# rssalessio/TZDDPC

Hardware: AMD Instinct MI355X
Metric: MPC steps/sec (batched trajectories), double-integrator N=20 (higher is better)
Workload: dtype f64

## Files before the change

### include/tzddpc.h

```cpp
#ifndef TZDDPC_H
#define TZDDPC_H

#include <stdint.h>

#ifdef __cplusplus
extern "C" {
#endif

#define TZ_ABI_VERSION 4

typedef enum tz_status {
  TZ_OK = 0,
  TZ_ERR_INVALID = -1,
  TZ_ERR_HIP = -2,
  TZ_ERR_UNSUPPORTED = -3
} tz_status;

enum {
  TZ_SOLVED = 0,
  TZ_MAX_ITER = 1,
  TZ_NUMERICAL = 2,
  TZ_INFEASIBLE = 3,
};

// ... 35 lines not shown
  int32_t pmax;
  const double* absCKpow;
  const double* absKCKpow;
  const int32_t* power;
  int32_t max_iter;
  double tol;
  double reg;
  double step_frac;
  const int32_t* shift_var;
  const int32_t* shift_row;
  const double* shift_xscale;
  const double* shift_lscale;
  const double* rec_c0;
  const double* rec_x0;
  const double* rec_y;
  int32_t plan_flags;
} tz_problem_desc;

enum {
  TZ_PLAN_UNFUSED = 1,
  TZ_PLAN_GENERAL_CHOLESKY = 2,
  TZ_PLAN_ITEM_GRAM = 4,
  TZ_PLAN_NO_STAIRCASE = 8,
  TZ_PLAN_ELL_PRODUCTS = 16
};

typedef struct tz_problem tz_problem;

int tz_abi_version(void);
const char* tz_last_error(void);
int tz_device_count(int* count);

int tz_identify_batch(int device, int32_t B, int32_t T, int32_t n, int32_t m, const double* u, const double* x,
                      const double* w_center, const double* K, int32_t k_shared,
                      double* C, double* s, double* sK, double* CK, int32_t* status, int mem);

int tz_specrad_batch(int device, int32_t S, int32_t n, int32_t ngen, const double* M0, const double* H, const double* beta,
                     double* rho, int32_t* status);
int tz_adversary_batch(int device, int32_t S, int32_t n, int32_t ngen, const double* M0, const double* H, const double* beta0,
                       int32_t max_iter, double* beta, double* fro, int32_t* steps);

typedef struct tz_genstack_desc {
  int32_t n, m, N, nseg;
  const int32_t* seg_ptr;
  const int32_t* src;
  const double* m0;
  const double* M;
// ... 33 lines not shown
               const double* A_true, const double* B_true, double* u_out, double* cost, int32_t* status);

int tz_problem_store_start(tz_problem* p, const double* xbar0, const double* e0);

int tz_problem_set_warm_shift(tz_problem* p, int32_t policy);
int tz_problem_set_warm_quiet(tz_problem* p, int32_t quiet_steps);

int tz_problem_set_stopping(tz_problem* p, double res_factor, double mu_factor);

int tz_problem_set_warm_push(tz_problem* p, double floor, double gain, double cap);

int tz_problem_reset_warm(tz_problem* p);

int tz_timing_enable(tz_problem* p, int enable);
int tz_timing_get(tz_problem* p, int kernel, double* total_ms, int64_t* launches);
int tz_ipm_work_get(tz_problem* p, int64_t* factorizations, int64_t* trajectory_solves, int64_t* max_factorizations_one_trajectory);

int tz_ipm_plan_info(tz_problem* p, int64_t* mfma_gram_per_iter, int64_t* mfma_chol_per_iter,
                     int64_t* mfma_issued_per_iter, int64_t* lds_bytes, int64_t* patch_bytes);

int tz_problem_plan_get(tz_problem* p, int32_t* fused, int32_t* one_wave_cholesky, int32_t* superstep_gram, int32_t* staircase,
                        int32_t* toeplitz);

int tz_debug_fetch(tz_problem* p, int32_t b, int what, double* out, int32_t capacity);

#ifdef __cplusplus
}
#endif
#endif
```

### tzddpc_amd/csrc/tz_ipm.hip.h

```cpp
#pragma once

#define TZ_MINWAVES 4
#define TZ_RLEV_CARRY_MAX 2
#ifndef TZ_RLEV_GATE
#define TZ_RLEV_GATE 1e6
#endif
#define TZ_SEED_VIOL_MAX 0.1
#define TZ_QROW 17
#define TZ_QSTR (4 * TZ_QROW)
struct IpmItem { int I0, q0, nq, kptr, klen; };

struct TzEll { int L, VL; const TzEllEnt* ent; const int* seg; const double* val; const unsigned short* idx; };
typedef __attribute__((address_space(1))) const char* tz_gptr;
typedef __attribute__((address_space(1))) const tz_d2* tz_gd2ptr;
__device__ inline double tz_ell_walk(const char* base_, unsigned lo, int L, unsigned stride, const double* in) {
  double a0 = 0.0, a1 = 0.0;
  const char* b = reinterpret_cast<const char*>(in);
  tz_gptr base = (tz_gptr)base_;
  int e = 0;
  for (; e + 3 < L; e += 4) {
    tz_gptr q0 = base, q1 = base + stride, q2 = base + 2 * (size_t)stride, q3 = base + 3 * (size_t)stride;
    asm volatile("" : "+s"(q0), "+s"(q1), "+s"(q2), "+s"(q3));
    const tz_d2 r0 = *(tz_gd2ptr)(q0 + lo), r1 = *(tz_gd2ptr)(q1 + lo), r2 = *(tz_gd2ptr)(q2 + lo), r3 = *(tz_gd2ptr)(q3 + lo);
    base += 4 * (size_t)stride;
// ... 35 lines not shown
  const int* smask;
  const double* q; const double* h;
  const int* prestatus;
  double* x; double* s; double* lam;
  int* status; int* iters;
  const int* prev_status;
  int* status_copy;
  int max_iter; double tol, reg, step_frac;
  double inv_mi;
  double mu_floor, tol_loose, step_frac_retry;
  double mu_tol;
  double tol_res;
  int warm_steps;
  int nell;
  int ntube;
  int shift_policy;
  int* shift_state;
  int shift_quiet;
  const int* sx; const int* sr; const double* sxs; const double* sls;
  int TS, ntile, gu;
  const struct TzGUnit* gunits; const int* gunit_ptr;
  int chol1;
  int ksplit;
  int warm; double warm_floor;
  double warm_gain, warm_cap;
  double aff_thr, aff_mu;
  unsigned long long* work;
  unsigned long long* prof;
  FuseParams F;
};

enum { PH_FORM = 0, PH_CHOL = 1, PH_SOLVE = 2, PH_GEMVT = 3, PH_GEMV = 4, PH_ELEM = 5, PH_TOTAL = 6, PH_CH_UPD = 8, PH_CH_DIAG = 9, PH_CH_PANEL = 10, PH_CH_BAR = 11, PH_PROLOGUE = 12, PH_EPILOGUE = 13, PH_GRAM_LOOP = 14, PH_GRAM_RED = 15, PH_GRAM_BAR = 16, PH_GRAM_RMW = 17, PH_TUBE = 18, PH_WARM = 19, PH_TOP = 20, PH_STEP = 21,
       PH_RD_A = 22, PH_RD_B = 23, PH_RD_C = 24, PH_EPI_A = 25, PH_EPI_B = 26, PH_MAPS_Q = 27, PH_WARM_A = 28, PH_WARM_B = 29, PH_TEST = 30, PH_T1 = 31, PH_T2 = 32, PH_T3 = 33, PH_COUNT = 34 };

__device__ inline int tz_qprefix(int I) {
  int a = I >> 2, b = I & 3;
  return (a + 1) * (2 * a + b);
}
__device__ inline int tz_hidx(int r, int c) {
  int I = r >> 2, J = c >> 2;
  return (tz_qprefix(I) + (J >> 2)) * TZ_QSTR + TZ_QROW * (r & 3) + 4 * (J & 3) + (c & 3);
}

__device__ inline int tz_tid() {
  int v = threadIdx.x;
  asm volatile("" : "+v"(v));
// ... 249 lines not shown
#pragma unroll
    for (int ii = 0; ii < 4; ++ii) {
      const int I = I0 + ii;
      if (I >= Tz) continue;
#pragma unroll
      for (int nn = 0; nn < 2; ++nn) {
        const int q = q0 + nn;
        if (nn >= nq || q > (I >> 2)) continue;
        const int r = 4 * I + i, c = 4 * (4 * q + blk) + j;
        double v = acc[ii][nn];
        if (c < p.nzp) v += p.P[(size_t)r * p.nzp + c];
        if (r == c) v = (r < p.nz) ? v + p.reg : 1.0;
        Hq[(tz_qprefix(I) + q) * TZ_QSTR + TZ_QROW * i + 4 * blk + j] = v;
      }
    }
  }
}

#define TZ_KS_TZ 10
__device__ inline double tz_sel4(int blk, double v0, double v1, double v2, double v3) {
  const double a = (blk & 1) ? v1 : v0, b = (blk & 1) ? v3 : v2;
  return (blk & 2) ? b : a;
}
struct TzGStage { double v[TZ_KS_TZ]; double w; int m; };

template <int N>
__device__ inline double tz_row_ror(double v) {
  const unsigned long long u = __builtin_bit_cast(unsigned long long, v);
  constexpr int ctrl = 0x120 + N;
  const unsigned lo = (unsigned)__builtin_amdgcn_mov_dpp((int)(unsigned)u, ctrl, 0xf, 0xf, true);
  const unsigned hi = (unsigned)__builtin_amdgcn_mov_dpp((int)(unsigned)(u >> 32), ctrl, 0xf, 0xf, true);
  return __builtin_bit_cast(double, ((unsigned long long)hi << 32) | lo);
}

template <int R0, int R1>
__device__ inline void tz_gram_rows(const IpmParams& p, double* Hq, const double* Pq, const double* wv, const int* sm, const int h, unsigned long long* pacc) {
  unsigned long long tq0 = pacc ? __builtin_amdgcn_s_memtime() : 0;
  const int lane = tz_tid() & 63;
  const int k = lane >> 4, blk = (lane >> 2) & 3, ij = lane & 3;
  const int Tz = p.Tz, Kc = p.Kc, S = (Kc + 3) >> 2;
  const unsigned rowbytes = (unsigned)(Tz + 1) * 128u;
  const char* gp = (const char*)p.Gp + (unsigned)(4 * k + ij) * 8u;
  double acc[R1 - R0][R1];
#pragma unroll
  for (int a = 0; a < R1 - R0; ++a)
#pragma unroll
    for (int J = 0; J < R1; ++J) acc[a][J] = 0.0;
  auto load = [&](int s, TzGStage& st) {
    int kc = 4 * s + blk; kc = (kc < Kc) ? kc : Kc;
    st.m = sm[s < S ? s : S];
    st.w = wv[4 * kc + k];
    const char* prow = gp + (size_t)kc * rowbytes;
#pragma unroll
    for (int J = 0; J < R1; ++J) st.v[J] = tz_ld_pinned((const double*)(prow + (unsigned)(J < Tz ? J : Tz) * 128u));
  };
  auto mma = [&](const TzGStage& st) {
    const int m = __builtin_amdgcn_readfirstlane(st.m);
#pragma unroll
    for (int I = R0; I < R1; ++I) {
      if ((m >> I) & 1) {
        const double a = st.v[I] * st.w;
#pragma unroll
        for (int J = 0; J <= I; ++J)
          if ((m >> J) & 1) acc[I - R0][J] = __builtin_amdgcn_mfma_f64_4x4x4f64(a, st.v[J], acc[I - R0][J], 0, 0, 0);
      }
    }
  };
  TzGStage s0, s1;
  load(h, s0);
  for (int s = h; s < S; s += 4) {
    load(s + 2, s1); mma(s0);
    load(s + 4, s0); mma(s1);
  }
  if (pacc) { unsigned long long t1 = __builtin_amdgcn_s_memtime(); pacc[PH_GRAM_LOOP] += t1 - tq0; tq0 = t1; }
  const int i = lane >> 4, j = lane & 3;
#pragma unroll
  for (int a = 0; a < R1 - R0; ++a)
#pragma unroll
    for (int J = 0; J < R1; ++J)
      if (J <= a + R0) { double v = acc[a][J]; v += tz_row_ror<4>(v); v += tz_row_ror<8>(v); acc[a][J] = v; }
  for (int hh = 0; hh < 2; ++hh) {
    if (h == hh) {
#pragma unroll
      for (int I = R0; I < R1; ++I) {
        if (I >= Tz) continue;
#pragma unroll
        for (int q = 0; q <= (I >> 2); ++q) {
          const double v0 = acc[I - R0][4 * q];
          const double v1 = (4 * q + 1 <= I) ? acc[I - R0][(4 * q + 1 <= I) ? 4 * q + 1 : 0] : 0.0;
          const double v2 = (4 * q + 2 <= I) ? acc[I - R0][(4 * q + 2 <= I) ? 4 * q + 2 : 0] : 0.0;
          const double v3 = (4 * q + 3 <= I) ? acc[I - R0][(4 * q + 3 <= I) ? 4 * q + 3 : 0] : 0.0;
          const int idx = (tz_qprefix(I) + q) * TZ_QSTR + TZ_QROW * i + 4 * blk + j;
          Hq[idx] = tz_sel4(blk, v0, v1, v2, v3) + ((hh == 0) ? Pq[idx] : Hq[idx]);
        }
      }
    }
    if (pacc) { unsigned long long t1 = __builtin_amdgcn_s_memtime(); pacc[hh == 0 ? PH_GRAM_RED : PH_GRAM_RMW] += t1 - tq0; tq0 = t1; }
    if (hh == 0) __syncthreads();
    if (pacc && hh == 0) { unsigned long long t1 = __builtin_amdgcn_s_memtime(); pacc[PH_GRAM_BAR] += t1 - tq0; tq0 = t1; }
  }
}

__device__ inline void tz_form_H_ksplit(const IpmParams& p, double* Hq, const double* Pq, const double* wv, const int* sm, unsigned long long* pacc) {
  const int wave = __builtin_amdgcn_readfirstlane(threadIdx.x >> 6);
  const int g = wave >> 1, h = wave & 1;
  if (p.Tz > 7) { if (g == 0) tz_gram_rows<0, 7>(p, Hq, Pq, wv, sm, h, pacc); else tz_gram_rows<7, 10>(p, Hq, Pq, wv, sm, h, pacc); }
  else          { if (g == 0) tz_gram_rows<0, 5>(p, Hq, Pq, wv, sm, h, pacc); else tz_gram_rows<5, 7>(p, Hq, Pq, wv, sm, h, pacc); }
}

__device__ inline void tz_gram(const IpmParams& p, double* Hq, const double* Pq, const double* wv, const int* kl, unsigned long long* pacc = nullptr) {
  if (p.ksplit) tz_form_H_ksplit(p, Hq, Pq, wv, kl, pacc);
  else tz_form_H(p, Hq, wv, kl);
}

__device__ inline void tz_sqrt_rsqrt(double d, double& sq, double& rs) {
  double y = __builtin_amdgcn_rsq(d);
  double g = d * y, h = 0.5 * y;
  double r = __builtin_fma(-h, g, 0.5);
  g = __builtin_fma(g, r, g); h = __builtin_fma(h, r, h);
  const double e = __builtin_fma(-g, g, d);
  g = __builtin_fma(e, h, g);
  double inv = h + h;
  const double e2 = __builtin_fma(-g, inv, 1.0);
  inv = __builtin_fma(e2, inv, inv);
  sq = g; rs = inv;
}

__device__ inline double tz_recip(double x) {
  double y = __builtin_amdgcn_rcp(x);
  y = __builtin_fma(__builtin_fma(-x, y, 1.0), y, y);
// ... 377 lines not shown
  double* thl = red + 34 + (p.nklist + 1) / 2;
  double* stl = thl + p.F.ntheta;
  double* pl = stl + 4 * TZ_NMAX;
  double* tbl = pl + p.nell;
  double* Pq = tbl + p.ntube;
  constexpr bool PARK = (MINW == 4);
  double* hL = Pq + (p.ksplit ? hsize : 0);
  double* gL = hL + mip;

  double s_[MAXR], l_[MAXR], h_[MAXR], gx_[MAXR];
#define TZ_H(k, r) (PARK ? hL[r] : h_[k])
#define TZ_GX(k, r) (PARK ? gL[r] : gx_[k])
#define TZ_SET_H(k, r, v) do { if (PARK) hL[r] = (v); else h_[k] = (v); } while (0)
#define TZ_ADD_GX(k, r, v) do { if (PARK) gL[r] += (v); else gx_[k] += (v); } while (0)
#define TZ_ROWS(k, r) _Pragma("unroll") for (int k = 0; k < MAXR; ++k) if (const int r = t + TZ_THREADS * k; r < mi)
  int rseg_[MAXR];
#pragma unroll
  for (int k = 0; k < MAXR; ++k) { const int r = t + TZ_THREADS * k; rseg_[k] = (r < mi) ? p.eg.seg[r] : 0; }
  const int ccol = (nzp <= 64 && t >= 64) ? (t < 128 ? t - 64 : nz) : t;
  const int cseg = (ccol < nz) ? p.et.seg[ccol] : 0;

  if (TT) { (void)kl; (void)Pq; }
  else if (p.ksplit) {
    for (int i = t; i <= ((p.Kc + 3) >> 2); i += TZ_THREADS) kl[i] = p.smask[i];
    for (int e = t; e < p.nquads * 64; e += TZ_THREADS) {
      const int qd = e >> 6;
      int I = 0;
      while (tz_qprefix(I + 1) <= qd) ++I;
      const int r = 4 * I + ((e >> 4) & 3), c = 4 * (4 * (qd - tz_qprefix(I)) + ((e >> 2) & 3)) + (e & 3);
      double v = (c < nzp) ? p.P[(size_t)r * nzp + c] : 0.0;
      if (r == c) v = (r < nz) ? v + p.reg : 1.0;
      Pq[qd * TZ_QSTR + TZ_QROW * ((e >> 4) & 3) + (e & 15)] = v;
    }
  }
  else for (int i = t; i < p.nklist; i += TZ_THREADS) kl[i] = p.klist[i];
  if (fused) {
    const int n = F0.fin.n, m = F0.fin.m, nv = F0.fin.N * m;
    const int n1 = (F0.tube.pmax + 1) * n * n, n2 = n1 + (F0.tube.pmax > 0 ? F0.tube.pmax : 1) * (n + m) * n;
    for (int i = t; i < n2; i += TZ_THREADS) tbl[i] = (i < n1) ? F0.tube.CKpow[i] : F0.tube.T[i - n1];
    double* ec = tbl + n2;
    for (int i = t; i < n * n; i += TZ_THREADS) { ec[i] = F0.plant.A[i]; ec[2 * n * m + n * n + n + i] = F0.fin.R2[i]; ec[2 * n * m + 2 * n * n + n + i] = F0.fin.Phi[(size_t)n * n + i]; }
    for (int i = t; i < n * m; i += TZ_THREADS) { ec[n * n + i] = F0.plant.Bm[i]; ec[n * n + n * m + i] = F0.plant.K[i]; }
    for (int i = t; i < n; i += TZ_THREADS) ec[n * n + 2 * n * m + i] = F0.fin.r1[i];
    for (int i = t; i < n * nv; i += TZ_THREADS) ec[3 * n * n + 2 * n * m + n + i] = F0.fin.Gam[(size_t)n * nv + i];
    for (int i = t; i < nv; i += TZ_THREADS) ec[3 * n * n + 2 * n * m + n + n * nv + i] = F0.fin.Dz[i];
    int* pwl = (int*)(ec + 3 * n * n + 2 * n * m + n + n * nv + nv);
    for (int i = t; i < F0.fin.N; i += TZ_THREADS) pwl[i] = F0.tube.power[i];
// ... 547 lines not shown
```

### tzddpc_amd/csrc/tzddpc_hip.hip

```cpp
#include "tz_kernels.hip.h"

static inline const char* tz_dev_getenv(const char* name) {
#if TZ_PROFILE
  return getenv(name);
#else
  (void)name;
  return nullptr;
#endif
}
#include "../../include/tzddpc.h"

#include <algorithm>
#include <cmath>
#include <cstdio>
#include <cstdlib>
#include <cstring>
#include <memory>
#include <numeric>
#include <string>
#include <vector>

static thread_local std::string g_err;

#define TZ_FAIL(code, ...) do { char _b[512]; snprintf(_b, sizeof(_b), __VA_ARGS__); g_err = _b; return (code); } while (0)
// ... 92 lines not shown
template <int R> ipm_fn_t ipm_pick_tt(int ncg, int w) {
  if (w >= 2) { switch (ncg) { case 1: case 2: return tz_ipm_kernel<R, 2, 2>; case 3: return tz_ipm_kernel<R, 3, 2>; default: return tz_ipm_kernel<R, 4, 2>; } }
  switch (ncg) { case 1: case 2: return tz_ipm_kernel<R, 2, 1>; case 3: return tz_ipm_kernel<R, 3, 1>; default: return tz_ipm_kernel<R, 4, 1>; }
}
ipm_fn_t ipm_kernel_for(int maxr, int ncg, int wgs_per_cu, bool& tt) {
#ifdef TZ_ONLY_SMALL
  tt = false;
  return (maxr == 1 && ncg == 1) ? tz_ipm_kernel<1, 1, TZ_MINWAVES> : nullptr;
#elif defined(TZ_ONLY_TT)
  tt = true; (void)wgs_per_cu;
  return tz_ipm_kernel<TZ_ONLY_TT>;
#else
  tt = (ncg >= 2 || maxr > 4);
  if (!tt) {
    switch (maxr) { case 1: return tz_ipm_kernel<1, 1, TZ_MINWAVES>; case 2: return tz_ipm_kernel<2, 1, TZ_MINWAVES>; case 3: return tz_ipm_kernel<3, 1, TZ_MINWAVES>; default: return tz_ipm_kernel<4, 1, TZ_MINWAVES>; }
  }
  switch (maxr) {
    case 1: return ipm_pick_tt<1>(ncg, wgs_per_cu); case 2: return ipm_pick_tt<2>(ncg, wgs_per_cu); case 3: return ipm_pick_tt<3>(ncg, wgs_per_cu);
    case 4: return ipm_pick_tt<4>(ncg, wgs_per_cu);
    case 5: return ncg <= 3 ? tz_ipm_kernel<5, 3, 1> : tz_ipm_kernel<5, 4, 1>;
    default: return ncg <= 3 ? tz_ipm_kernel<6, 3, 1> : tz_ipm_kernel<6, 4, 1>;
  }
#endif
}

}

struct tz_problem {
  int device = 0;
  int n = 0, m = 0, N = 0, nz = 0, mi = 0, ntheta = 0, npar = 0, nc_rows = 0, pmax = 0;
  int nzp = 0, mip = 0, Tz = 0, Kc = 0, nquads = 0, nklist = 0, nP = 0;
  int max_iter = 40;
  double tol = 1e-10, reg = 1e-12, step_frac = 0.99, cost_scale = 1.0, r0 = 0.0;
  DevBuf<double> P, G, Gt, Gp, act_scale, Dz, Phi, Gam, r1, R2, CK, DK, K, CKpow, Ttube, par_lo, par_hi, rec0, recx, recy;
  DevBuf<int> power, row_of, klist, item_ptr, smask, shift_var, shift_row;
  DevBuf<double> shift_xs, shift_ls;
  int shift_policy = 0;
  int shift_quiet = 16;
  bool have_shift = false;
  DevBuf<IpmItem> items;
  DevCsr q, h, par;
  DevEll eg, et;
  int nell = 0;
  size_t lds_bytes = 0;
  int64_t mfma_gram = 0, mfma_chol = 0, mfma_issued = 0;
  int Bcap = 0;
// ... 4 lines not shown
  hipStream_t stream = nullptr;
  bool own_stream = false;
  bool timing = false;
  std::vector<std::pair<hipEvent_t, hipEvent_t>> ev_pool[K_COUNT];
  size_t ev_used[K_COUNT] = {0, 0, 0, 0};
  double t_ms[K_COUNT] = {0, 0, 0, 0};
  int64_t t_count[K_COUNT] = {0, 0, 0, 0};
  int lastB = 0;
  bool prof = false;
  bool have_prev = false; int prevB = 0;
  DevBuf<double> ref_x, ref_lam;
  bool have_ref = false;
  double warm_floor = 1e-8, warm_gain = 1.0, warm_cap = 1e300, mu_factor = 1e-3, res_factor = 100.0, aff_thr = 0.99, aff_mu = 1e-3;
  bool warm_enabled = true;
  int ntube = 0;
  bool tt = false;
  int TS = 16, ntile = 0, gu = 0;
  size_t hsize = 0;
  DevBuf<TzGUnit> gunits; DevBuf<int> gunit_ptr;
  DevBuf<int> vpos;
  std::vector<int> permc, permr;
  bool chol1 = false;
  bool ksplit = false;
  bool fuse_enabled = true;
  bool staircase = false;
  bool toeplitz = false;
  bool lean_epilogue = false;
  struct tz_genstack* tube_stack = nullptr;
  DevBuf<double> ts_zeta, ts_c, ts_rx, ts_ru;  int ts_cap = 0;
  int maxr = 1, ncg = 1;
  void (*ipm_fn)(IpmParams) = nullptr;
  DevBuf<unsigned long long> prof_buf, work_buf;
};

extern "C" int tube_stack_theta(tz_problem* p, int B, const double* d_e0, hipStream_t st);

namespace {

int ensure_workspace(tz_problem* p, int B) {
  if (B <= p->Bcap) return TZ_OK;
  TZ_HIP(hipSetDevice(p->device));
  size_t b = (size_t)B;
  TZ_HIP(p->theta.alloc(b * p->ntheta));
  TZ_HIP(p->qv.alloc(b * p->nz));
  TZ_HIP(p->hv.alloc(b * p->mi));
  TZ_HIP(p->x.alloc(b * p->nz));
// ... 37 lines not shown
    if (!p->timing) return;
    if (p->ev_used[k] == p->ev_pool[k].size()) {
      if (p->ev_pool[k].size() >= 4096) drain_timing_one(p, k);
      else {
        hipEvent_t a, b;
        if (hipEventCreate(&a) != hipSuccess || hipEventCreate(&b) != hipSuccess) return;
        p->ev_pool[k].push_back({a, b});
      }
    }
    e0 = p->ev_pool[k][p->ev_used[k]].first; e1 = p->ev_pool[k][p->ev_used[k]].second;
    p->ev_used[k]++;
    (void)hipEventRecord(e0, p->stream);
  }
  ~Timer() { if (e1) (void)hipEventRecord(e1, p->stream); }
};

void drain_timing(tz_problem* p) {
  for (int k = 0; k < K_COUNT; ++k) drain_timing_one(p, k);
}

IpmParams ipm_params(tz_problem* p, int B, int* d_status, int* d_iters, bool warm, bool track_prev) {
  IpmParams ip{};
  ip.B = B; ip.nz = p->nz; ip.mi = p->mi; ip.nzp = p->nzp; ip.mip = p->mip; ip.Tz = p->Tz; ip.Kc = p->Kc; ip.nquads = p->nquads;
  ip.P = p->P.p; ip.Gp = p->Gp.p; ip.items = p->items.p; ip.item_ptr = p->item_ptr.p; ip.klist = p->klist.p; ip.smask = p->smask.p; ip.eg = p->eg.view(); ip.et = p->et.view(); ip.nell = p->nell;
  ip.q = p->qv.p; ip.h = p->hv.p; ip.prestatus = p->prestatus.p; ip.x = p->x.p; ip.s = p->s.p; ip.lam = p->lam.p;
  ip.status = d_status; ip.iters = d_iters ? d_iters : p->iters.p;
  ip.max_iter = p->max_iter; ip.tol = p->tol; ip.reg = p->reg; ip.step_frac = p->step_frac; ip.mu_tol = p->tol * p->mu_factor; ip.tol_res = p->tol * p->res_factor;
  ip.inv_mi = 1.0 / p->mi; ip.mu_floor = 1e-3 * ip.mu_tol; ip.tol_loose = 1e3 * p->tol; ip.step_frac_retry = std::min(p->step_frac, 0.99);
  ip.prof = p->prof ? p->prof_buf.p : nullptr;
  ip.work = p->timing ? p->work_buf.p : nullptr;
  ip.TS = p->TS; ip.ntile = p->ntile; ip.gu = p->gu; ip.gunits = p->gunits.p; ip.gunit_ptr = p->gunit_ptr.p;
  ip.nklist = p->nklist; ip.nP = p->nP; ip.ksplit = p->ksplit ? 1 : 0; ip.chol1 = p->chol1 ? 1 : 0; ip.ntube = p->ntube;
  ip.shift_policy = p->have_shift ? p->shift_policy : 0; ip.shift_quiet = p->shift_quiet;
  ip.shift_state = p->shift_state.p;
  ip.sx = p->shift_var.p; ip.sr = p->shift_row.p; ip.sxs = p->shift_xs.p; ip.sls = p->shift_ls.p;
  ip.warm = warm ? 1 : 0; ip.warm_floor = p->warm_floor;
  ip.warm_gain = p->warm_gain; ip.warm_cap = p->warm_cap; ip.aff_thr = p->aff_thr; ip.aff_mu = p->aff_mu;
  ip.prev_status = warm ? p->prev_status.p : nullptr;
  ip.status_copy = track_prev ? p->prev_status.p : nullptr;
  ip.F.on = 0;
  return ip;
}

struct StepStrides { size_t w, u, x, cost; };
int launch_step_fused(tz_problem* p, int B, double* d_x, double* d_xbar, double* d_e, const double* d_w, size_t w_stride,
                      const double* d_A, const double* d_Bm, double* d_u, size_t u_stride, double* d_xout, size_t x_stride,
                      double* d_cost, size_t cost_stride, int* d_status, int* d_sticky, bool warm,
                      int nsteps = 1, StepStrides ss = StepStrides{0, 0, 0, 0}, bool sticky_fresh = false) {
  p->lastB = B;
  Timer tm(p, K_IPM);
  IpmParams ip = ipm_params(p, B, d_status, p->iters.p, warm, true);
  FuseParams& F = ip.F;
  F.on = 1; F.npar = p->npar; F.ntheta = p->ntheta; F.lean_epilogue = p->lean_epilogue ? 1 : 0; F.sticky_fresh = sticky_fresh ? 1 : 0;
  F.nsteps = nsteps; F.warm_steps = p->warm_enabled ? 1 : 0; ip.warm_steps = F.warm_steps;
  F.w_step = ss.w; F.u_step = ss.u; F.x_step = ss.x; F.cost_step = ss.cost;
// ... 693 lines not shown
        p->TS = c.TS; wgs_per_cu = c.wgs; p->lds_bytes = need;
        if (c.small) { p->eg.swap(eg_small); p->nell = nell_small; }
        placed = true; break;
      }
    }
    if (!placed) { TZ_HIP(need_small()); return fail_lds(lds_for(16, nell_small)); }
    p->hsize = (size_t)p->ntile * p->TS;
    bool ttk = false;
    p->ipm_fn = ipm_kernel_for(p->maxr, p->ncg, wgs_per_cu, ttk);
    if (p->maxr > 4) wgs_per_cu = 1;
    plan(TZ_TT_GU(wgs_per_cu));
    if (best_units.empty()) TZ_FAIL(TZ_ERR_UNSUPPORTED, "no Gram plan for Tz=%d", Tz);
    p->gu = best_u;
    TZ_HIP(p->gunits.upload(best_units)); TZ_HIP(p->gunit_ptr.upload(best_ptr));
    p->mfma_gram = (int64_t)best_span; p->mfma_chol = (int64_t)Tz * Tz * Tz / 24; p->mfma_issued = p->mfma_gram * TZ_NWAVES + p->mfma_chol;
  } else {
    p->ksplit = (p->Tz <= TZ_KS_TZ);
    p->chol1 = (p->Tz <= 16);
    if (d->plan_flags & TZ_PLAN_GENERAL_CHOLESKY) p->chol1 = false;
    if (d->plan_flags & TZ_PLAN_ITEM_GRAM) p->ksplit = false;
    if (const char* e = tz_dev_getenv("TZ_CHOL1")) { if (e[0] == '0') p->chol1 = false; }
    if (const char* e = tz_dev_getenv("TZ_KSPLIT")) { if (e[0] == '0') p->ksplit = false; }
    p->hsize = (size_t)p->nquads * TZ_QSTR;
    p->lds_bytes = tz_ipm_lds_doubles(p->hsize, 0, Tz, nzp, mip, p->nklist, p->ntheta, p->ksplit ? 1 : 0, p->ntube, p->nell, 1) * sizeof(double);
    if (p->lds_bytes > LDS_MAX) return fail_lds(p->lds_bytes);
    wgs_per_cu = (int)(LDS_MAX / std::max<size_t>(p->lds_bytes, 1));
    bool ttk = false;
    p->ipm_fn = ipm_kernel_for(p->maxr, p->ncg, wgs_per_cu, ttk);
  }
  if (!p->ipm_fn) TZ_FAIL(TZ_ERR_UNSUPPORTED, "this development build (TZ_ONLY_SMALL) carries only the mi <= 256, nz <= 64 kernel");
  {
    bool ttk = false;
    (void)ipm_kernel_for(p->maxr, p->ncg, wgs_per_cu, ttk);
    if (ttk != p->tt) TZ_FAIL(TZ_ERR_UNSUPPORTED, "kernel class and table format disagree (development build?)");
  }
  TZ_HIP(hipFuncSetAttribute((const void*)p->ipm_fn, hipFuncAttributeMaxDynamicSharedMemorySize, (int)p->lds_bytes));
  if (const char* e = tz_dev_getenv("TZ_PROF")) { p->prof = (e[0] == '1'); }
  if (p->prof && !TZ_PROFILE) TZ_FAIL(TZ_ERR_INVALID, "TZ_PROF=1 needs the diagnostic build of the library (libtzddpc_hip_prof.so)");
  if (const char* e = tz_dev_getenv("TZ_WARM")) { p->warm_enabled = (e[0] != '0'); }
  if (d->plan_flags & TZ_PLAN_UNFUSED) p->fuse_enabled = false;
  if (const char* e = tz_dev_getenv("TZ_FUSE")) { p->fuse_enabled = (e[0] != '0'); }
  if ((size_t)std::max(p->pmax, 1) * p->n > p->hsize) p->fuse_enabled = false;
  {
    auto envd = [](const char* name, double lo, bool lo_open, double hi, double& dst) -> bool {
      const char* e = tz_dev_getenv(name);
      if (!e) return true;
// ... 302 lines not shown

int tz_ipm_work_get(tz_problem* p, int64_t* factorizations, int64_t* trajectory_solves, int64_t* max_factorizations_one_trajectory) {
  if (!p || !factorizations || !trajectory_solves) TZ_FAIL(TZ_ERR_INVALID, "null argument");
  TZ_HIP(hipSetDevice(p->device));
  TZ_HIP(hipStreamSynchronize(p->stream));
  unsigned long long h[3];
  TZ_HIP(hipMemcpy(h, p->work_buf.p, sizeof(h), hipMemcpyDeviceToHost));
  *factorizations = (int64_t)h[0]; *trajectory_solves = (int64_t)h[1];
  if (max_factorizations_one_trajectory) *max_factorizations_one_trajectory = (int64_t)h[2];
  return TZ_OK;
}

int tz_ipm_plan_info(tz_problem* p, int64_t* mfma_gram_per_iter, int64_t* mfma_chol_per_iter, int64_t* mfma_issued_per_iter,
                     int64_t* lds_bytes, int64_t* patch_bytes) {
  if (!p) TZ_FAIL(TZ_ERR_INVALID, "null problem");
  if (mfma_gram_per_iter) *mfma_gram_per_iter = p->mfma_gram;
  if (mfma_chol_per_iter) *mfma_chol_per_iter = p->mfma_chol;
  if (mfma_issued_per_iter) *mfma_issued_per_iter = p->mfma_issued;
  if (lds_bytes) *lds_bytes = (int64_t)p->lds_bytes;
  if (patch_bytes) *patch_bytes = (int64_t)p->Gp.n * 8;
  return TZ_OK;
}

int tz_problem_plan_get(tz_problem* p, int32_t* fused, int32_t* one_wave_cholesky, int32_t* superstep_gram, int32_t* staircase, int32_t* toeplitz) {
  if (!p) TZ_FAIL(TZ_ERR_INVALID, "null problem");
  if (fused) *fused = p->fuse_enabled ? 1 : 0;
  if (one_wave_cholesky) *one_wave_cholesky = p->chol1 ? 1 : 0;
  if (superstep_gram) *superstep_gram = p->ksplit ? 1 : 0;
  if (staircase) *staircase = p->staircase ? 1 : 0;
  if (toeplitz) *toeplitz = p->toeplitz ? 1 : 0;
  return TZ_OK;
}

int tz_debug_fetch(tz_problem* p, int32_t b, int what, double* out, int32_t capacity) {
  if (!p || !out) TZ_FAIL(TZ_ERR_INVALID, "null argument");
  if (b < 0 || b >= p->lastB) TZ_FAIL(TZ_ERR_INVALID, "trajectory %d outside the last batch (%d)", b, p->lastB);
  TZ_HIP(hipSetDevice(p->device));
  TZ_HIP(hipStreamSynchronize(p->stream));
  const double* src = nullptr; int len = 0;
  switch (what) {
    case 0: src = p->theta.p + (size_t)b * p->ntheta; len = p->ntheta; break;
    case 1: src = p->qv.p + (size_t)b * p->nz; len = p->nz; break;
    case 2: src = p->hv.p + (size_t)b * p->mi; len = p->mi; break;
    case 3: src = p->x.p + (size_t)b * p->nz; len = p->nz; break;
    case 4: src = p->s.p + (size_t)b * p->mi; len = p->mi; break;
    case 5: src = p->lam.p + (size_t)b * p->mi; len = p->mi; break;
// ... 30 lines not shown
```

### tzddpc_amd/native.py

```python
from __future__ import annotations

import ctypes as C
import os
from typing import Optional

import numpy as np

TZ_ABI_VERSION = 4
TZ_MEM_HOST, TZ_MEM_DEVICE = 0, 1
TZ_SOLVED, TZ_MAX_ITER, TZ_NUMERICAL, TZ_INFEASIBLE = 0, 1, 2, 3

_HERE = os.path.dirname(os.path.abspath(__file__))
LIB_PATH = os.path.join(_HERE, "lib", "libtzddpc_hip_prof.so" if os.environ.get("TZ_PROF") == "1" else "libtzddpc_hip.so")
if os.environ.get("TZ_LIB"):
    LIB_PATH = os.path.abspath(os.environ["TZ_LIB"])

_dp = C.POINTER(C.c_double)
_ip = C.POINTER(C.c_int32)


class NativeError(RuntimeError):
    pass


class AffMap(C.Structure):
    _fields_ = [("rows", C.c_int32), ("ptr", _ip), ("col", _ip), ("val", _dp), ("c0", _dp)]


class ProblemDesc(C.Structure):
    _fields_ = [
        ("abi_version", C.c_int32), ("n", C.c_int32), ("m", C.c_int32), ("N", C.c_int32),
        ("nz", C.c_int32), ("mi", C.c_int32), ("ntheta", C.c_int32),
        ("P", _dp), ("G", _dp), ("q", AffMap), ("h", AffMap), ("par", AffMap),
        ("par_lo", _dp), ("par_hi", _dp),
        ("cost_scale", C.c_double), ("r0", C.c_double), ("r1", _dp), ("R2", _dp),
        ("Dz", _dp), ("Phi", _dp), ("Gam", _dp),
        ("nc_rows", C.c_int32), ("row_of", _ip), ("act_scale", _dp),
        ("CK", _dp), ("DK", _dp), ("K", _dp), ("pmax", C.c_int32), ("absCKpow", _dp), ("absKCKpow", _dp), ("power", _ip),
        ("max_iter", C.c_int32), ("tol", C.c_double), ("reg", C.c_double), ("step_frac", C.c_double),
        ("shift_var", _ip), ("shift_row", _ip), ("shift_xscale", _dp), ("shift_lscale", _dp),
        ("rec_c0", _dp), ("rec_x0", _dp), ("rec_y", _dp),
        ("plan_flags", C.c_int32),
    ]


TZ_PLAN_UNFUSED, TZ_PLAN_GENERAL_CHOLESKY, TZ_PLAN_ITEM_GRAM, TZ_PLAN_NO_STAIRCASE, TZ_PLAN_ELL_PRODUCTS = 1, 2, 4, 8, 16


class GenstackDesc(C.Structure):
    _fields_ = [("n", C.c_int32), ("m", C.c_int32), ("N", C.c_int32), ("nseg", C.c_int32), ("seg_ptr", _ip), ("src", _ip),
                ("m0", _dp), ("M", _dp), ("c0", _dp), ("cE", _dp), ("cZ", _dp), ("K", _dp)]


_lib = None


def build_hint() -> str:
    return ("build it with `python -c 'import __graft_entry__ as g; g.build()'` "
            "(python -c 'import __graft_entry__ as g; g.build()', i.e. hipcc --offload-arch=gfx950 -shared -fPIC tzddpc_amd/csrc/tzddpc_hip.hip)")


def lib():
    global _lib
    if _lib is not None:
        return _lib
    try:
        import torch
    except Exception:
        pass
# ... 26 lines not shown
    L.tz_genstack_intervals.argtypes = [vp, C.c_int32, vp, vp, vp, vp, vp, C.POINTER(C.c_double), C.c_int]
    L.tz_genstack_values.argtypes = [vp, C.c_int32, C.c_int32, vp, vp, vp, C.c_int]
    L.tz_genstack_info.argtypes = [vp] + [C.POINTER(C.c_int64)] * 3
    for nm in ("tz_problem_attach_tube_stack", "tz_genstack_create", "tz_genstack_destroy", "tz_genstack_intervals", "tz_genstack_values", "tz_genstack_info"):
        getattr(L, nm).restype = C.c_int
    L.tz_problem_reset_warm.argtypes = [vp]
    L.tz_problem_store_start.argtypes = [vp, vp, vp]
    L.tz_problem_store_start.restype = C.c_int
    L.tz_problem_attach_tube_stack.argtypes = [vp, vp]
    L.tz_problem_attach_tube_stack.restype = C.c_int
    L.tz_problem_set_stopping.argtypes = [vp, C.c_double, C.c_double]
    L.tz_problem_set_stopping.restype = C.c_int
    L.tz_problem_set_warm_quiet.argtypes = [vp, C.c_int32]
    L.tz_problem_set_warm_quiet.restype = C.c_int
    L.tz_problem_set_warm_push.argtypes = [vp, C.c_double, C.c_double, C.c_double]
    L.tz_problem_set_warm_push.restype = C.c_int
    L.tz_problem_set_warm_shift.argtypes = [vp, C.c_int32]
    L.tz_timing_enable.argtypes = [vp, C.c_int]
    L.tz_timing_get.argtypes = [vp, C.c_int, C.POINTER(C.c_double), C.POINTER(C.c_int64)]
    L.tz_ipm_plan_info.argtypes = [vp] + [C.POINTER(C.c_int64)] * 5
    L.tz_ipm_work_get.argtypes = [vp, C.POINTER(C.c_int64), C.POINTER(C.c_int64), C.POINTER(C.c_int64)]
    L.tz_problem_plan_get.argtypes = [vp] + [C.POINTER(C.c_int32)] * 5
    L.tz_problem_plan_get.restype = C.c_int
    L.tz_debug_fetch.argtypes = [vp, C.c_int32, C.c_int, vp, C.c_int32]
    for name in ("tz_device_count", "tz_problem_create", "tz_problem_destroy", "tz_problem_set_stream", "tz_problem_sync",
                 "tz_solve_batch", "tz_simulate_batch", "tz_mpc_step", "tz_mpc_run", "tz_timing_enable", "tz_timing_get",
                 "tz_ipm_plan_info", "tz_ipm_work_get", "tz_debug_fetch", "tz_problem_reset_warm", "tz_problem_set_warm_shift"):
        getattr(L, name).restype = C.c_int
    if L.tz_abi_version() != TZ_ABI_VERSION:
        raise NativeError(f"ABI mismatch: library {L.tz_abi_version()} vs binding {TZ_ABI_VERSION}")
    _lib = L
    return L


EXPORTED_SYMBOLS = ("tz_abi_version", "tz_last_error", "tz_device_count", "tz_problem_create", "tz_problem_destroy", "tz_problem_plan_get", "tz_problem_store_start",
                    "tz_problem_set_stream", "tz_problem_sync", "tz_solve_batch", "tz_simulate_batch", "tz_mpc_step", "tz_mpc_run",
                    "tz_timing_enable", "tz_timing_get", "tz_ipm_plan_info", "tz_ipm_work_get", "tz_debug_fetch",
                    "tz_problem_set_warm_shift", "tz_problem_set_stopping", "tz_problem_set_warm_quiet", "tz_problem_set_warm_push", "tz_problem_reset_warm", "tz_identify_batch", "tz_specrad_batch", "tz_adversary_batch",
                    "tz_problem_attach_tube_stack", "tz_genstack_create", "tz_genstack_destroy", "tz_genstack_intervals", "tz_genstack_values", "tz_genstack_info")


def check(rc: int, what: str):
    if rc < 0:
        raise NativeError(f"{what} failed ({rc}): {lib().tz_last_error().decode(errors='replace')}")
    return rc


def device_count() -> int:
    n = C.c_int(0)
    check(lib().tz_device_count(C.byref(n)), "tz_device_count")
    return n.value


def identify_batch(device: int, u: np.ndarray, x: np.ndarray, w_center: np.ndarray, K: Optional[np.ndarray] = None):
    u = np.ascontiguousarray(u, dtype=np.float64); x = np.ascontiguousarray(x, dtype=np.float64)
    if u.ndim == 2:
        u = u[None]; x = x[None]
    B, T, m = u.shape
# ... 206 lines not shown

    def timing_enable(self, on: bool = True):
        check(lib().tz_timing_enable(self._h, int(on)), "tz_timing_enable")

    def timing_get(self, kernel: int):
        ms = C.c_double(0); cnt = C.c_int64(0)
        check(lib().tz_timing_get(self._h, kernel, C.byref(ms), C.byref(cnt)), "tz_timing_get")
        return ms.value, cnt.value

    def work_get(self):
        a, b, c = C.c_int64(0), C.c_int64(0), C.c_int64(0)
        check(lib().tz_ipm_work_get(self._h, C.byref(a), C.byref(b), C.byref(c)), "tz_ipm_work_get")
        return dict(factorizations=a.value, trajectory_solves=b.value, max_factorizations_one_trajectory=c.value)

    def plan_info(self):
        a, b, i, c, d = (C.c_int64(0) for _ in range(5))
        check(lib().tz_ipm_plan_info(self._h, C.byref(a), C.byref(b), C.byref(i), C.byref(c), C.byref(d)), "tz_ipm_plan_info")
        f = [C.c_int32(0) for _ in range(5)]
        check(lib().tz_problem_plan_get(self._h, *[C.byref(v) for v in f]), "tz_problem_plan_get")
        return dict(mfma_gram_per_iter=a.value, mfma_chol_per_iter=b.value, mfma_issued_per_iter=i.value,
                    lds_bytes=c.value, patch_bytes=d.value, fused=bool(f[0].value), chol1=bool(f[1].value), ksplit=bool(f[2].value),
                    staircase=bool(f[3].value), toeplitz=bool(f[4].value))

    def last_iterations(self, B: int) -> np.ndarray:
        out = np.empty(int(B))
        n = check(lib().tz_debug_fetch(self._h, 0, 7, out.ctypes.data_as(C.c_void_p), int(B)), "tz_debug_fetch")
        return out[:n].astype(np.int64)

    def debug_fetch(self, b: int, what: int) -> np.ndarray:
        cap = max(self.nz, self.mi, self.ntheta, 64)
        out = np.empty(cap)
        n = check(lib().tz_debug_fetch(self._h, int(b), int(what), out.ctypes.data_as(C.c_void_p), cap), "tz_debug_fetch")
        return out[:n].copy()


class GenStack:

    def __init__(self, device: int, st):
        d = GenstackDesc()
        keep = []
        d.n, d.m, d.N, d.nseg = int(st.n), int(st.m), int(st.N), int(st.nseg)
        sp = _i32(st.seg_ptr); sr = _i32(st.src if st.src.size else np.zeros(1)); keep += [sp, sr]
        d.seg_ptr = _ptr(sp, _ip); d.src = _ptr(sr, _ip)
        for name in ("m0", "M", "c0", "cE", "K"):
            a = _f64(getattr(st, name))
            if a.size == 0:
# ... 52 lines not shown
```

Before: 101.2 million.

## Pair mirror-image constraint rows in the Gram build to halve MFMA work

Detects constraint rows of G that are equal up to sign (e.g. upper/lower bounds) and packs each pair into one slot of the k-split Gram build. It uses w_a+w_b for blocks where the signs agree and w_a-w_b for blocks where they differ, so each pair costs one MFMA update instead of two. This adds a host planning pass, a new packed G buffer and pair table, and extra LDS for the table. The plan is only taken when LDS occupancy is not reduced, and the kernel gains a template branch plus two extra weight loads per stage.

Result: slower. 99.57 million, median of 2 (-1.6%).

```diff
diff --git a/include/tzddpc.h b/include/tzddpc.h
--- a/include/tzddpc.h
+++ b/include/tzddpc.h
@@ -81,7 +81,8 @@
   TZ_PLAN_GENERAL_CHOLESKY = 2,
   TZ_PLAN_ITEM_GRAM = 4,
   TZ_PLAN_NO_STAIRCASE = 8,
-  TZ_PLAN_ELL_PRODUCTS = 16
+  TZ_PLAN_ELL_PRODUCTS = 16,
+  TZ_PLAN_NO_ROW_PAIRS = 32
 };
 
 typedef struct tz_problem tz_problem;
@@ -161,6 +162,8 @@
 int tz_problem_plan_get(tz_problem* p, int32_t* fused, int32_t* one_wave_cholesky, int32_t* superstep_gram, int32_t* staircase,
                         int32_t* toeplitz);
 
+int tz_problem_row_pairs(tz_problem* p, int32_t* pairs);
+
 int tz_debug_fetch(tz_problem* p, int32_t b, int what, double* out, int32_t capacity);
 
 #ifdef __cplusplus
diff --git a/tzddpc_amd/csrc/tz_ipm.hip.h b/tzddpc_amd/csrc/tz_ipm.hip.h
--- a/tzddpc_amd/csrc/tz_ipm.hip.h
+++ b/tzddpc_amd/csrc/tz_ipm.hip.h
@@ -81,6 +81,7 @@
   const struct TzGUnit* gunits; const int* gunit_ptr;
   int chol1;
   int ksplit;
+  int pairs;
   int warm; double warm_floor;
   double warm_gain, warm_cap;
   double aff_thr, aff_mu;
@@ -376,7 +377,7 @@
   const double a = (blk & 1) ? v1 : v0, b = (blk & 1) ? v3 : v2;
   return (blk & 2) ? b : a;
 }
-struct TzGStage { double v[TZ_KS_TZ]; double w; int m; };
+struct TzGStage { double v[TZ_KS_TZ]; double w; int m; int nx; };
 
 template <int N>
 __device__ inline double tz_row_ror(double v) {
@@ -387,7 +388,7 @@
   return __builtin_bit_cast(double, ((unsigned long long)hi << 32) | lo);
 }
 
-template <int R0, int R1>
+template <int R0, int R1, bool PAIRS>
 __device__ inline void tz_gram_rows(const IpmParams& p, double* Hq, const double* Pq, const double* wv, const int* sm, const int h, unsigned long long* pacc) {
   unsigned long long tq0 = pacc ? __builtin_amdgcn_s_memtime() : 0;
   const int lane = tz_tid() & 63;
@@ -400,23 +401,35 @@
   for (int a = 0; a < R1 - R0; ++a)
 #pragma unroll
     for (int J = 0; J < R1; ++J) acc[a][J] = 0.0;
+  const int* sw = sm + S + 1 + 4 * blk + k;
   auto load = [&](int s, TzGStage& st) {
     int kc = 4 * s + blk; kc = (kc < Kc) ? kc : Kc;
     st.m = sm[s < S ? s : S];
-    st.w = wv[4 * kc + k];
+    if constexpr (PAIRS) {
+      st.nx = sw[16 * (s < S ? s : S)];
+    } else {
+      st.w = wv[4 * kc + k];
+    }
     const char* prow = gp + (size_t)kc * rowbytes;
 #pragma unroll
     for (int J = 0; J < R1; ++J) st.v[J] = tz_ld_pinned((const double*)(prow + (unsigned)(J < Tz ? J : Tz) * 128u));
   };
   auto mma = [&](const TzGStage& st) {
-    const int m = __builtin_amdgcn_readfirstlane(st.m);
+    const int mx = __builtin_amdgcn_readfirstlane(st.m);
+    const int m = PAIRS ? (mx & 0xffff) : mx, x = PAIRS ? (mx >> 16) : 0;
+    double w = st.w, wm = 0.0;
+    if constexpr (PAIRS) { const double wa = wv[st.nx & 0xffff], wb = wv[st.nx >> 16]; w = wa + wb; wm = wa - wb; }
 #pragma unroll
     for (int I = R0; I < R1; ++I) {
       if ((m >> I) & 1) {
-        const double a = st.v[I] * st.w;
+        const double a = st.v[I] * w;
+        const double am = PAIRS ? st.v[I] * wm : a;
 #pragma unroll
         for (int J = 0; J <= I; ++J)
-          if ((m >> J) & 1) acc[I - R0][J] = __builtin_amdgcn_mfma_f64_4x4x4f64(a, st.v[J], acc[I - R0][J], 0, 0, 0);
+          if ((m >> J) & 1) {
+            const double aij = (PAIRS && (((x >> I) ^ (x >> J)) & 1)) ? am : a;
+            acc[I - R0][J] = __builtin_amdgcn_mfma_f64_4x4x4f64(aij, st.v[J], acc[I - R0][J], 0, 0, 0);
+          }
       }
     }
   };
@@ -458,8 +471,13 @@
 __device__ inline void tz_form_H_ksplit(const IpmParams& p, double* Hq, const double* Pq, const double* wv, const int* sm, unsigned long long* pacc) {
   const int wave = __builtin_amdgcn_readfirstlane(threadIdx.x >> 6);
   const int g = wave >> 1, h = wave & 1;
-  if (p.Tz > 7) { if (g == 0) tz_gram_rows<0, 7>(p, Hq, Pq, wv, sm, h, pacc); else tz_gram_rows<7, 10>(p, Hq, Pq, wv, sm, h, pacc); }
-  else          { if (g == 0) tz_gram_rows<0, 5>(p, Hq, Pq, wv, sm, h, pacc); else tz_gram_rows<5, 7>(p, Hq, Pq, wv, sm, h, pacc); }
+  if (p.pairs) {
+    if (p.Tz > 7) { if (g == 0) tz_gram_rows<0, 7, true>(p, Hq, Pq, wv, sm, h, pacc); else tz_gram_rows<7, 10, true>(p, Hq, Pq, wv, sm, h, pacc); }
+    else          { if (g == 0) tz_gram_rows<0, 5, true>(p, Hq, Pq, wv, sm, h, pacc); else tz_gram_rows<5, 7, true>(p, Hq, Pq, wv, sm, h, pacc); }
+  } else {
+    if (p.Tz > 7) { if (g == 0) tz_gram_rows<0, 7, false>(p, Hq, Pq, wv, sm, h, pacc); else tz_gram_rows<7, 10, false>(p, Hq, Pq, wv, sm, h, pacc); }
+    else          { if (g == 0) tz_gram_rows<0, 5, false>(p, Hq, Pq, wv, sm, h, pacc); else tz_gram_rows<5, 7, false>(p, Hq, Pq, wv, sm, h, pacc); }
+  }
 }
 
 __device__ inline void tz_gram(const IpmParams& p, double* Hq, const double* Pq, const double* wv, const int* kl, unsigned long long* pacc = nullptr) {
@@ -883,7 +901,7 @@
 
   if (TT) { (void)kl; (void)Pq; }
   else if (p.ksplit) {
-    for (int i = t; i <= ((p.Kc + 3) >> 2); i += TZ_THREADS) kl[i] = p.smask[i];
+    for (int i = t, n = (((p.Kc + 3) >> 2) + 1) * (p.pairs ? 17 : 1); i < n; i += TZ_THREADS) kl[i] = p.smask[i];
     for (int e = t; e < p.nquads * 64; e += TZ_THREADS) {
       const int qd = e >> 6;
       int I = 0;
diff --git a/tzddpc_amd/csrc/tzddpc_hip.hip b/tzddpc_amd/csrc/tzddpc_hip.hip
--- a/tzddpc_amd/csrc/tzddpc_hip.hip
+++ b/tzddpc_amd/csrc/tzddpc_hip.hip
@@ -138,6 +138,81 @@
     default: return ncg <= 3 ? tz_ipm_kernel<6, 3, 1> : tz_ipm_kernel<6, 4, 1>;
   }
 #endif
+}
+
+struct RowPairPlan { int npairs = 0, S = 0; int64_t mfma = 0; std::vector<double> Gq; std::vector<int> tab; };
+RowPairPlan row_pair_plan(const std::vector<double>& G, int mi, int nz, int nzp, int Tz) {
+  RowPairPlan pl;
+  std::vector<int> supp((size_t)mi, 0), partner((size_t)mi, -1), flip((size_t)mi, 0);
+  for (int r = 0; r < mi; ++r) for (int c = 0; c < nz; ++c) if (G[(size_t)r * nzp + c] != 0.0) supp[r] |= 1 << (c >> 2);
+  std::vector<std::pair<std::vector<uint64_t>, int>> keys((size_t)mi);
+  for (int r = 0; r < mi; ++r) {
+    keys[r].second = r;
+    for (int c = 0; c < nz; ++c) {
+      const double v = G[(size_t)r * nzp + c];
+      if (v != 0.0) { uint64_t u; const double a = std::fabs(v); std::memcpy(&u, &a, 8); keys[r].first.push_back((uint64_t)c); keys[r].first.push_back(u); }
+    }
+  }
+  std::sort(keys.begin(), keys.end());
+  for (size_t i0 = 0; i0 < keys.size();) {
+    size_t i1 = i0;
+    while (i1 < keys.size() && keys[i1].first == keys[i0].first) ++i1;
+    for (size_t i = i0; i < i1 && !keys[i0].first.empty(); ++i) {
+      const int a = keys[i].second;
+      if (partner[a] >= 0) continue;
+      for (size_t j = i + 1; j < i1; ++j) {
+        const int b = keys[j].second;
+        if (partner[b] >= 0) continue;
+        int neg = 0, pos = 0;
+        for (int c = 0; c < nz; ++c) {
+          const double va = G[(size_t)a * nzp + c];
+          if (va != 0.0) { if ((va < 0.0) != (G[(size_t)b * nzp + c] < 0.0)) neg |= 1 << (c >> 2); else pos |= 1 << (c >> 2); }
+        }
+        if (neg & pos) continue;
+        partner[a] = b; partner[b] = a; flip[a] = neg; ++pl.npairs;
+        break;
+      }
+    }
+    i0 = i1;
+  }
+  if (pl.npairs == 0) return pl;
+  std::vector<int> items, rest;
+  for (int r = 0; r < mi; ++r) if (partner[r] < 0 || partner[r] > r) items.push_back(r);
+  std::vector<std::vector<int>> steps; std::vector<int> xs;
+  while (!items.empty()) {
+    std::vector<int> cur; rest.clear();
+    int X = 0, K = 0;
+    for (int r : items) {
+      if ((int)cur.size() == 16) { rest.push_back(r); continue; }
+      if (partner[r] < 0) { cur.push_back(r); continue; }
+      const int T = supp[r], com = T & K;
+      int f = flip[r];
+      const int dd = (f ^ X) & com;
+      if (dd != 0 && dd != com) { rest.push_back(r); continue; }
+      if (com != 0 && dd == com) f ^= T;
+      X = (X & ~T) | (f & T); K |= T;
+      cur.push_back(r);
+    }
+    steps.push_back(cur); xs.push_back(X); items.swap(rest);
+  }
+  const int S = (int)steps.size();
+  pl.S = S;
+  pl.Gq.assign((size_t)(4 * S + 1) * (Tz + 1) * 16, 0.0);
+  pl.tab.assign((size_t)(S + 1) * 17, mi | (mi << 16));
+  for (int s = 0; s <= S; ++s) pl.tab[s] = 0;
+  for (int s = 0; s < S; ++s) {
+    int m = 0;
+    for (int l = 0; l < (int)steps[s].size(); ++l) {
+      const int r = steps[s][l], kc = 4 * s + (l >> 2), k = l & 3;
+      for (int c = 0; c < nz; ++c) pl.Gq[((size_t)kc * (Tz + 1) + (c >> 2)) * 16 + 4 * k + (c & 3)] = G[(size_t)r * nzp + c];
+      pl.tab[S + 1 + 16 * s + l] = r | ((partner[r] >= 0 ? partner[r] : mi) << 16);
+      m |= supp[r];
+    }
+    pl.tab[s] = m | ((xs[s] & m) << 16);
+    const int64_t cnt = __builtin_popcount(m);
+    pl.mfma += cnt * (cnt + 1) / 2;
+  }
+  return pl;
 }
 
 }
@@ -188,6 +263,8 @@
   std::vector<int> permc, permr;
   bool chol1 = false;
   bool ksplit = false;
+  int npairs = 0, gram_kc = 0;
+  DevBuf<double> Gq; DevBuf<int> ptab;
   bool fuse_enabled = true;
   bool staircase = false;
   bool toeplitz = false;
@@ -271,7 +348,7 @@
 IpmParams ipm_params(tz_problem* p, int B, int* d_status, int* d_iters, bool warm, bool track_prev) {
   IpmParams ip{};
   ip.B = B; ip.nz = p->nz; ip.mi = p->mi; ip.nzp = p->nzp; ip.mip = p->mip; ip.Tz = p->Tz; ip.Kc = p->Kc; ip.nquads = p->nquads;
-  ip.P = p->P.p; ip.Gp = p->Gp.p; ip.items = p->items.p; ip.item_ptr = p->item_ptr.p; ip.klist = p->klist.p; ip.smask = p->smask.p; ip.eg = p->eg.view(); ip.et = p->et.view(); ip.nell = p->nell;
+  ip.P = p->P.p; ip.Gp = p->npairs ? p->Gq.p : p->Gp.p; ip.items = p->items.p; ip.item_ptr = p->item_ptr.p; ip.klist = p->klist.p; ip.smask = p->npairs ? p->ptab.p : p->smask.p; ip.eg = p->eg.view(); ip.et = p->et.view(); ip.nell = p->nell;
   ip.q = p->qv.p; ip.h = p->hv.p; ip.prestatus = p->prestatus.p; ip.x = p->x.p; ip.s = p->s.p; ip.lam = p->lam.p;
   ip.status = d_status; ip.iters = d_iters ? d_iters : p->iters.p;
   ip.max_iter = p->max_iter; ip.tol = p->tol; ip.reg = p->reg; ip.step_frac = p->step_frac; ip.mu_tol = p->tol * p->mu_factor; ip.tol_res = p->tol * p->res_factor;
@@ -279,7 +356,8 @@
   ip.prof = p->prof ? p->prof_buf.p : nullptr;
   ip.work = p->timing ? p->work_buf.p : nullptr;
   ip.TS = p->TS; ip.ntile = p->ntile; ip.gu = p->gu; ip.gunits = p->gunits.p; ip.gunit_ptr = p->gunit_ptr.p;
-  ip.nklist = p->nklist; ip.nP = p->nP; ip.ksplit = p->ksplit ? 1 : 0; ip.chol1 = p->chol1 ? 1 : 0; ip.ntube = p->ntube;
+  if (p->npairs) ip.Kc = p->gram_kc;
+  ip.nklist = p->nklist; ip.nP = p->nP; ip.ksplit = p->ksplit ? 1 : 0; ip.pairs = p->npairs ? 1 : 0; ip.chol1 = p->chol1 ? 1 : 0; ip.ntube = p->ntube;
   ip.shift_policy = p->have_shift ? p->shift_policy : 0; ip.shift_quiet = p->shift_quiet;
   ip.shift_state = p->shift_state.p;
   ip.sx = p->shift_var.p; ip.sr = p->shift_row.p; ip.sxs = p->shift_xs.p; ip.sls = p->shift_ls.p;
@@ -1019,6 +1097,16 @@
     if (const char* e = tz_dev_getenv("TZ_CHOL1")) { if (e[0] == '0') p->chol1 = false; }
     if (const char* e = tz_dev_getenv("TZ_KSPLIT")) { if (e[0] == '0') p->ksplit = false; }
     p->hsize = (size_t)p->nquads * TZ_QSTR;
+    if (p->ksplit && !(d->plan_flags & TZ_PLAN_NO_ROW_PAIRS) && mi < 0xffff) {
+      RowPairPlan rp = row_pair_plan(G, mi, nz, nzp, Tz);
+      const int nk = std::max(p->nklist, (int)rp.tab.size());
+      auto lds = [&](int nkl) { return tz_ipm_lds_doubles(p->hsize, 0, Tz, nzp, mip, nkl, p->ntheta, 1, p->ntube, p->nell, 1) * sizeof(double); };
+      if (rp.npairs > 0 && LDS_MAX / lds(nk) >= LDS_MAX / lds(p->nklist)) {
+        TZ_HIP(p->Gq.upload(rp.Gq)); TZ_HIP(p->ptab.upload(rp.tab));
+        p->npairs = rp.npairs; p->gram_kc = 4 * rp.S; p->nklist = nk;
+        p->mfma_gram = rp.mfma; p->mfma_issued = rp.mfma + p->mfma_chol;
+      }
+    }
     p->lds_bytes = tz_ipm_lds_doubles(p->hsize, 0, Tz, nzp, mip, p->nklist, p->ntheta, p->ksplit ? 1 : 0, p->ntube, p->nell, 1) * sizeof(double);
     if (p->lds_bytes > LDS_MAX) return fail_lds(p->lds_bytes);
     wgs_per_cu = (int)(LDS_MAX / std::max<size_t>(p->lds_bytes, 1));
@@ -1367,6 +1455,12 @@
   return TZ_OK;
 }
 
+int tz_problem_row_pairs(tz_problem* p, int32_t* pairs) {
+  if (!p || !pairs) TZ_FAIL(TZ_ERR_INVALID, "null argument");
+  *pairs = p->npairs;
+  return TZ_OK;
+}
+
 int tz_problem_plan_get(tz_problem* p, int32_t* fused, int32_t* one_wave_cholesky, int32_t* superstep_gram, int32_t* staircase, int32_t* toeplitz) {
   if (!p) TZ_FAIL(TZ_ERR_INVALID, "null problem");
   if (fused) *fused = p->fuse_enabled ? 1 : 0;
diff --git a/tzddpc_amd/native.py b/tzddpc_amd/native.py
--- a/tzddpc_amd/native.py
+++ b/tzddpc_amd/native.py
@@ -44,7 +44,7 @@
     ]
 
 
-TZ_PLAN_UNFUSED, TZ_PLAN_GENERAL_CHOLESKY, TZ_PLAN_ITEM_GRAM, TZ_PLAN_NO_STAIRCASE, TZ_PLAN_ELL_PRODUCTS = 1, 2, 4, 8, 16
+TZ_PLAN_UNFUSED, TZ_PLAN_GENERAL_CHOLESKY, TZ_PLAN_ITEM_GRAM, TZ_PLAN_NO_STAIRCASE, TZ_PLAN_ELL_PRODUCTS, TZ_PLAN_NO_ROW_PAIRS = 1, 2, 4, 8, 16, 32
 
 
 class GenstackDesc(C.Structure):
@@ -117,6 +117,8 @@
     L.tz_ipm_work_get.argtypes = [vp, C.POINTER(C.c_int64), C.POINTER(C.c_int64), C.POINTER(C.c_int64)]
     L.tz_problem_plan_get.argtypes = [vp] + [C.POINTER(C.c_int32)] * 5
     L.tz_problem_plan_get.restype = C.c_int
+    L.tz_problem_row_pairs.argtypes = [vp, C.POINTER(C.c_int32)]
+    L.tz_problem_row_pairs.restype = C.c_int
     L.tz_debug_fetch.argtypes = [vp, C.c_int32, C.c_int, vp, C.c_int32]
     for name in ("tz_device_count", "tz_problem_create", "tz_problem_destroy", "tz_problem_set_stream", "tz_problem_sync",
                  "tz_solve_batch", "tz_simulate_batch", "tz_mpc_step", "tz_mpc_run", "tz_timing_enable", "tz_timing_get",
@@ -128,7 +130,7 @@
     return L
 
 
-EXPORTED_SYMBOLS = ("tz_abi_version", "tz_last_error", "tz_device_count", "tz_problem_create", "tz_problem_destroy", "tz_problem_plan_get", "tz_problem_store_start",
+EXPORTED_SYMBOLS = ("tz_abi_version", "tz_last_error", "tz_device_count", "tz_problem_create", "tz_problem_destroy", "tz_problem_plan_get", "tz_problem_row_pairs", "tz_problem_store_start",
                     "tz_problem_set_stream", "tz_problem_sync", "tz_solve_batch", "tz_simulate_batch", "tz_mpc_step", "tz_mpc_run",
                     "tz_timing_enable", "tz_timing_get", "tz_ipm_plan_info", "tz_ipm_work_get", "tz_debug_fetch",
                     "tz_problem_set_warm_shift", "tz_problem_set_stopping", "tz_problem_set_warm_quiet", "tz_problem_set_warm_push", "tz_problem_reset_warm", "tz_identify_batch", "tz_specrad_batch", "tz_adversary_batch",
@@ -381,6 +383,11 @@
                     lds_bytes=c.value, patch_bytes=d.value, fused=bool(f[0].value), chol1=bool(f[1].value), ksplit=bool(f[2].value),
                     staircase=bool(f[3].value), toeplitz=bool(f[4].value))
 
+    def row_pairs(self) -> int:
+        v = C.c_int32(0)
+        check(lib().tz_problem_row_pairs(self._h, C.byref(v)), "tz_problem_row_pairs")
+        return int(v.value)
+
     def last_iterations(self, B: int) -> np.ndarray:
         out = np.empty(int(B))
         n = check(lib().tz_debug_fetch(self._h, 0, 7, out.ctypes.data_as(C.c_void_p), int(B)), "tz_debug_fetch")
```
